# YPares/gaast

Hardware: AMD Instinct MI355X
Metric: full-MV geometric products/sec (dim n); achieved HBM GB/s vs roofline (higher is better)
Workload: dtype f32; 1 GPU; R^12 full MV x MV geometric product, f32 (BASELINE configs[2]); dim=12, batch_per_gpu=65536, global_batch=65536

## Files before the change

gaast_amd/csrc/device/kernels_dense.hip.hpp:

```cpp
#pragma once
#include "kernels_common.hip.hpp"


namespace gaast {

template <typename T>
struct DenseArgs {
    const T* left;
    const T* right;
    T* out;
    int64_t left_stride, right_stride, out_stride;
    const uint32_t* left_map;
    const uint32_t* right_map;
    int left_count, right_count;
    int left_full, right_full;
    int left_contig, right_contig;
    const int32_t* out_map;
    int canon_left, canon_right;
    int n;
    uint32_t neg_hi, zero_hi;
    uint32_t neg_lo;
    int beta;
    const T* left_scale;
    const T* right_scale;
// ... 275 lines not shown
        asm("v_pk_fma_f32 %0, %1, %2, %0 op_sel:[1,1,0] op_sel_hi:[1,0,1]" : "+v"(c) : "v"(a), "v"(b));
    else if constexpr (X == 1 && NL == 1 && NH == 0)
        asm("v_pk_fma_f32 %0, %1, %2, %0 op_sel:[1,1,0] op_sel_hi:[1,0,1] neg_lo:[1,0,0]" : "+v"(c) : "v"(a), "v"(b));
    else if constexpr (X == 1 && NL == 0 && NH == 1)
        asm("v_pk_fma_f32 %0, %1, %2, %0 op_sel:[1,1,0] op_sel_hi:[1,0,1] neg_hi:[1,0,0]" : "+v"(c) : "v"(a), "v"(b));
    else
        asm("v_pk_fma_f32 %0, %1, %2, %0 op_sel:[1,1,0] op_sel_hi:[1,0,1] neg_lo:[1,0,0] neg_hi:[1,0,0]" : "+v"(c) : "v"(a), "v"(b));
}

template <bool ODD, bool NEGLO, int IDX>
__device__ __forceinline__ void gp_block16_pk(const float2v (&A2)[8], const float2v (&B2)[8], float2v (&C2)[8]) {
    if constexpr (IDX < 128) {
        constexpr int a = IDX >> 3, j = IDX & 7, c0 = 2 * j;
        constexpr int b_lo = a ^ c0, b_hi = a ^ c0 ^ 1;
        constexpr int nl = lo_reorder_parity(a, b_lo) ^ (ODD ? (__builtin_popcount(b_lo) & 1) : 0) ^
                           (NEGLO ? (__builtin_popcount(a & b_lo) & 1) : 0);
        constexpr int nh = lo_reorder_parity(a, b_hi) ^ (ODD ? (__builtin_popcount(b_hi) & 1) : 0) ^
                           (NEGLO ? (__builtin_popcount(a & b_hi) & 1) : 0);
        pk_fma_sel<(a & 1), nl, nh>(C2[j], A2[a >> 1], B2[b_lo >> 1]);
        gp_block16_pk<ODD, NEGLO, IDX + 1>(A2, B2, C2);
    }
}

template <typename T>
struct BlockStep;

template <>
struct BlockStep<float> {
    float2v C2[8];
    __device__ __forceinline__ void init() {
#pragma unroll
        for (int i = 0; i < 8; ++i) C2[i] = float2v{0.f, 0.f};
    }
    template <bool ODD, bool NEGLO>
    __device__ __forceinline__ void step(const float* As, const float* Bs, int a_hi, int b_hi, float sgn) {
        const int sa = (a_hi >> 2) & 3, sb = (b_hi >> 2) & 3;
        const float4v* ap = reinterpret_cast<const float4v*>(As + (a_hi << 4));
        const float4v* bp = reinterpret_cast<const float4v*>(Bs + (b_hi << 4));
        float2v A2[8], B2[8];
        const float2v s2 = float2v{sgn, sgn};
#pragma unroll
        for (int q = 0; q < 4; ++q) {
            const float4v va = ap[q ^ sa];
            const float4v vb = bp[q ^ sb];
            A2[2 * q] = float2v{va.x, va.y};
            A2[2 * q + 1] = float2v{va.z, va.w};
            B2[2 * q] = float2v{vb.x, vb.y} * s2;
            B2[2 * q + 1] = float2v{vb.z, vb.w} * s2;
        }
        gp_block16_pk<ODD, NEGLO, 0>(A2, B2, C2);
    }
    __device__ __forceinline__ float get(int i) const { return (i & 1) ? C2[i >> 1].y : C2[i >> 1].x; }
};

template <>
struct BlockStep<double> {
    double C[16];
    __device__ __forceinline__ void init() {
#pragma unroll
        for (int i = 0; i < 16; ++i) C[i] = 0.0;
    }
    template <bool ODD, bool NEGLO>
    __device__ __forceinline__ void step(const double* As, const double* Bs, int a_hi, int b_hi, double sgn) {
        const int sa = (a_hi >> 2) & 3, sb = (b_hi >> 2) & 3;
        const double2v* ap = reinterpret_cast<const double2v*>(As + (a_hi << 4));
        const double2v* bp = reinterpret_cast<const double2v*>(Bs + (b_hi << 4));
        double A[16], B[16];
#pragma unroll
        for (int q = 0; q < 4; ++q) {
            const double2v a0 = ap[2 * (q ^ sa)], a1 = ap[2 * (q ^ sa) + 1];
            const double2v b0 = bp[2 * (q ^ sb)], b1 = bp[2 * (q ^ sb) + 1];
            A[4 * q + 0] = a0.x; A[4 * q + 1] = a0.y; A[4 * q + 2] = a1.x; A[4 * q + 3] = a1.y;
            B[4 * q + 0] = b0.x * sgn; B[4 * q + 1] = b0.y * sgn; B[4 * q + 2] = b1.x * sgn; B[4 * q + 3] = b1.y * sgn;
        }
        gp_block16<double, ODD, NEGLO>(A, B, C);
    }
    __device__ __forceinline__ double get(int i) const { return C[i]; }
};

template <typename T, bool DEGENERATE, int THREADS, bool NEGLO, bool SCALED = false, bool CHAINED = false>
__global__ __launch_bounds__(THREADS) void k_gp_dense(DenseArgs<T> p) {
    const T* const left_scale = SCALED ? p.left_scale : nullptr;
    const T* const right_scale = SCALED ? p.right_scale : nullptr;
    const T* const out_scale = SCALED ? p.out_scale : nullptr;
    extern __shared__ __attribute__((aligned(16))) unsigned char smem_raw[];
    T* smem = reinterpret_cast<T*>(smem_raw);
    const int n = p.n;
    const int N = 1 << n;
    const int hbits = n - 4;
    const int LPI = 1 << hbits;
    const int IPB = THREADS >> hbits;
    const int item_stride = 2 * N + (IPB > 1 ? 4 : 0);
    const int tid = threadIdx.x;
    const T zero = T(0);
    const int64_t num_groups = (p.batch + IPB - 1) / IPB;

    const int it = tid >> hbits;
    const int c_hi = tid & (LPI - 1);
    int32_t om[16];
#pragma unroll
    for (int i = 0; i < 16; ++i) om[i] = p.out_map[(c_hi << 4) + i];

    for (int64_t grp = blockIdx.x; grp < num_groups; grp += gridDim.x) {
        const int64_t item0 = grp * IPB;
        const int nitems = int(p.batch - item0 < IPB ? p.batch - item0 : IPB);
        {
            if (!p.left_full || !p.right_full) {
                for (int i = tid; i < nitems * item_stride; i += THREADS) smem[i] = zero;
                __syncthreads();
            }
            if constexpr (CHAINED)
                stage_from_list<T, THREADS>(p, item0, nitems, smem, item_stride, smem + p.pre_scratch, tid);
            else
                stage_operands<T, THREADS>(p.left + item0 * p.left_stride, p.left_stride, p.left_map, p.left_count, p.left_contig,
                                           p.canon_left, smem, item_stride, nitems, tid, left_scale);
            stage_operands<T, THREADS>(p.right + item0 * p.right_stride, p.right_stride, p.right_map, p.right_count,
                                       p.right_contig, p.canon_right, smem + N, item_stride, nitems, tid, right_scale);
        }
        __syncthreads();

        if (it < nitems) {
            const T* As = smem + it * item_stride;
            const T* Bs = As + N;
            BlockStep<T> acc;
            acc.init();

            auto one_step = [&](auto odd_tag, int a_hi) {
                constexpr bool ODD = decltype(odd_tag)::value;
                uint32_t sp = uint32_t(a_hi) >> 1;
                sp ^= sp >> 1;
                sp ^= sp >> 2;
                sp ^= sp >> 4;
                sp ^= sp >> 8;
                const uint32_t M = sp ^ (uint32_t(a_hi) & p.neg_hi);
                const uint32_t u = (__builtin_popcount(uint32_t(a_hi) & sp) ^
                                    __builtin_popcount(uint32_t(a_hi) & p.neg_hi)) & 1u;
                const uint32_t sbit = (u ^ uint32_t(__builtin_popcount(uint32_t(c_hi) & M))) & 1u;
                T sgn = sbit ? T(-1) : T(1);
                if (DEGENERATE) {
                    if (uint32_t(a_hi) & ~uint32_t(c_hi) & p.zero_hi) sgn = zero;
                }
                acc.template step<ODD, NEGLO>(As, Bs, a_hi, a_hi ^ c_hi, sgn);
            };
            const int half = LPI >> 1;
            for (int i = 0; i < half; ++i) one_step(std::false_type{}, (i << 1) | (__builtin_popcount(uint32_t(i)) & 1));
            for (int i = 0; i < half; ++i) one_step(std::true_type{}, (i << 1) | ((__builtin_popcount(uint32_t(i)) & 1) ^ 1));

            T* orow = p.out + (item0 + it) * p.out_stride;
#pragma unroll
            for (int i = 0; i < 16; ++i) store_result<T>(orow, om[i], acc.get(i), p.beta, out_scale, (c_hi << 4) + i);
        }
        __syncthreads();
    }
}


__device__ __forceinline__ constexpr int lo5_reorder_parity(int a, int b) {
    int par = 0;
    for (int p = 1; p < 5; ++p)
        if ((a >> p) & 1)
            for (int q = 0; q < p; ++q) par ^= (b >> q) & 1;
    return par;
}

__device__ __forceinline__ int mfma_b_pos(int m) {
    const int x = m >> 5, k = m & 31;
    const int lq = ((k & 1) << 2) | (k >> 3);
    return (x << 5) | (((lq ^ (x >> 1)) & 7) << 2) | ((k >> 1) & 3);
}

template <bool DEGENERATE, int THREADS, bool SCALED = false, bool CHAINED = false>
__global__ __launch_bounds__(THREADS) void k_gp_mfma32(DenseArgs<float> p) {
    const float* const left_scale = SCALED ? p.left_scale : nullptr;
    const float* const right_scale = SCALED ? p.right_scale : nullptr;
    const float* const out_scale = SCALED ? p.out_scale : nullptr;
    extern __shared__ __attribute__((aligned(16))) unsigned char smem_raw[];
    float* smem = reinterpret_cast<float*>(smem_raw);
    const int n = p.n;
    const int N = 1 << n;
    const int hbits = n - 5;
    const int H = 1 << hbits;
    const int WPI = H >> 5;
    const int IPB = (THREADS >> 6) / WPI;
    const int item_stride = 2 * N;
    const int tid = threadIdx.x;
    const int64_t item0 = int64_t(blockIdx.x) * IPB;
    const int nitems = int(p.batch - item0 < IPB ? p.batch - item0 : IPB);

    if (!p.left_full || !p.right_full) {
        for (int i = tid; i < nitems * item_stride; i += THREADS) smem[i] = 0.f;
        __syncthreads();
    }
    {
        if constexpr (CHAINED)
            stage_from_list<float, THREADS>(p, item0, nitems, smem, item_stride, smem + p.pre_scratch, tid);
        else
            stage_operands<float, THREADS>(p.left + item0 * p.left_stride, p.left_stride, p.left_map, p.left_count, p.left_contig,
                                       p.canon_left, smem, item_stride, nitems, tid, left_scale);
        stage_operands<float, THREADS>(p.right + item0 * p.right_stride, p.right_stride, p.right_map, p.right_count,
                                       p.right_contig, p.canon_right, smem + N, item_stride, nitems, tid, right_scale);
    }
    __syncthreads();

    const int wave = tid >> 6, lane = tid & 63;
    const int it = wave / WPI, tile = wave - it * WPI;
    if (it < nitems) {
        const float* As = smem + it * item_stride;
        const float* Bs = As + N;
        const int i = lane & 31, h = lane >> 5;
        const int c_hi = (tile << 5) | i;

        uint32_t amask[16];
        uint32_t aoff[16];
#pragma unroll
        for (int s2 = 0; s2 < 16; ++s2) {
            const int k = 2 * s2 + h;
            const int a_lo = i ^ k;
            int par = __builtin_popcount(uint32_t(a_lo & k) & p.neg_lo) & 1;
            for (int pp = 1; pp < 5; ++pp)
                if ((a_lo >> pp) & 1) par ^= __builtin_popcount(k & ((1 << pp) - 1)) & 1;
            amask[s2] = uint32_t(par) << 31;
            aoff[s2] = uint32_t(a_lo) << 2;
        }

        float16v acc;
#pragma unroll
        for (int r = 0; r < 16; ++r) acc[r] = 0.f;

        const unsigned char* As_b = reinterpret_cast<const unsigned char*>(As);
        const unsigned char* Bs_b = reinterpret_cast<const unsigned char*>(Bs);
        uint32_t bq[4];
#pragma unroll
        for (int q = 0; q < 4; ++q) bq[q] = (uint32_t(c_hi) << 7) | (uint32_t((((h << 2) | q) ^ (c_hi >> 1)) & 7) << 4);
        const uint32_t c_hi_u = uint32_t(c_hi) | 0x8000u;
        auto one_step = [&](int a_hi) {
            uint32_t sp = uint32_t(a_hi) >> 1;
            sp ^= sp >> 1;
            sp ^= sp >> 2;
            sp ^= sp >> 4;
            sp ^= sp >> 8;
            const uint32_t M = sp ^ (uint32_t(a_hi) & p.neg_hi);
            const uint32_t u = (__builtin_popcount(uint32_t(a_hi) & sp) ^
                                __builtin_popcount(uint32_t(a_hi) & p.neg_hi)) & 1u;
            const uint32_t bmask = uint32_t(__builtin_popcount(c_hi_u & (M | (u << 15)))) << 31;
            float bscale = 1.f;
            if (DEGENERATE) {
                if (uint32_t(a_hi) & ~uint32_t(c_hi) & p.zero_hi) bscale = 0.f;
            }
            float bv[16];
            const uint32_t sx = (uint32_t(a_hi) << 7) | (uint32_t((a_hi >> 1) & 7) << 4);
#pragma unroll
            for (int q = 0; q < 4; ++q) {
                const float4v v = *reinterpret_cast<const float4v*>(Bs_b + (bq[q] ^ sx));
                bv[4 * q + 0] = v.x; bv[4 * q + 1] = v.y; bv[4 * q + 2] = v.z; bv[4 * q + 3] = v.w;
            }
            const uint32_t abase = uint32_t(a_hi) << 7;
#pragma unroll
            for (int s2 = 0; s2 < 16; ++s2) {
                float a = *reinterpret_cast<const float*>(As_b + abase + aoff[s2]);
                a = __uint_as_float(__float_as_uint(a) ^ amask[s2]);
                float b = __uint_as_float(__float_as_uint(bv[s2]) ^ bmask);
                if (DEGENERATE) b *= bscale;
                acc = __builtin_amdgcn_mfma_f32_32x32x2f32(a, b, acc, 0, 0, 0);
            }
        };
        const int half = H >> 1;
        for (int t2 = 0; t2 < half; ++t2) one_step((t2 << 1) | (__builtin_popcount(uint32_t(t2)) & 1));
#pragma unroll
        for (int s2 = 0; s2 < 16; ++s2)
            amask[s2] ^= uint32_t((__builtin_popcount(uint32_t(s2)) + h) & 1) << 31;
        for (int t2 = 0; t2 < half; ++t2) one_step((t2 << 1) | ((__builtin_popcount(uint32_t(t2)) & 1) ^ 1));

        float* orow = p.out + (item0 + it) * p.out_stride;
        const int32_t* om = p.out_map + (c_hi << 5);
#pragma unroll
        for (int r = 0; r < 16; ++r) {
            const int c_lo = (r & 3) + 8 * (r >> 2) + 4 * h;
            store_result<float>(orow, om[c_lo], acc[r], p.beta, out_scale, (c_hi << 5) + c_lo);
        }
    }
}

template <int THREADS>
__device__ __forceinline__ void lds_barrier() {
    if (THREADS <= 64) {
        __builtin_amdgcn_wave_barrier();
        asm volatile("" ::: "memory");
    } else {
        asm volatile("s_waitcnt lgkmcnt(0)\n\ts_barrier" ::: "memory");
    }
}

typedef __attribute__((address_space(3))) unsigned char lds_u8;
typedef uint32_t uint4v __attribute__((ext_vector_type(4)));

__device__ __forceinline__ uint32_t xor3(uint32_t a, uint32_t b, uint32_t c) {
#if __has_builtin(__builtin_amdgcn_bitop3_b32)
    return __builtin_amdgcn_bitop3_b32(a, b, c, 0x96);
#else
    return a ^ b ^ c;
#endif
}

__device__ __forceinline__ constexpr int mfma16_k(int t) {
    constexpr int order[16] = {0, 3, 5, 6, 9, 10, 12, 15, 1, 2, 4, 7, 8, 11, 13, 14};
    return order[t];
}

template <bool DEGENERATE, int NDIM, bool SCALED = false, bool CHAINED = false>
__global__ __launch_bounds__(NDIM == 13 ? 512 : 256, NDIM <= 11 ? 2 : 1) void k_gp_mfma32p(DenseArgs<float> p) {
    const float* const left_scale = SCALED ? p.left_scale : nullptr;
    const float* const right_scale = SCALED ? p.right_scale : nullptr;
    const float* const out_scale = SCALED ? p.out_scale : nullptr;
    extern __shared__ __attribute__((aligned(16))) unsigned char smem_raw[];
    float* smem = reinterpret_cast<float*>(smem_raw);
    lds_u8* lds = (lds_u8*)smem_raw;
    constexpr int n = NDIM;
    constexpr int THREADS = NDIM == 13 ? 512 : 256;
    constexpr int N = 1 << n;
    constexpr int H = 1 << (n - 5);
    constexpr int WPI = H >> 5;
    constexpr int IPB = (THREADS >> 6) / WPI;
    constexpr int item_stride = 4 * N;
    constexpr uint32_t NEG = uint32_t(N) << 2;
    constexpr int PR = N / 4;
    constexpr int MPR = PR / THREADS;
    constexpr int ROWS = 2 * IPB;
    static_assert(MPR * ROWS == 8, "eight 16-byte pieces per thread and group");
    const int tid = threadIdx.x;
    const int64_t num_groups = (p.batch + IPB - 1) / IPB;
    const bool fast = !SCALED && !CHAINED && p.left_contig && p.right_contig && p.left_full && p.right_full;

    if (tid < 16) smem[IPB * item_stride + tid] = 0.f;

    uint32_t mw[2][MPR * 4];
    float4 pf[8];
    auto fetch = [&](int64_t g) {
        const int64_t it0 = g * IPB;
        const int cnt = int(p.batch - it0 < IPB ? p.batch - it0 : IPB);
#pragma unroll
        for (int r = 0; r < ROWS; ++r) {
            const int k = r % IPB;
            if (k < cnt) {
                const float* row = r < IPB ? p.left + (it0 + k) * p.left_stride : p.right + (it0 + k) * p.right_stride;
#pragma unroll
                for (int m = 0; m < MPR; ++m) pf[r * MPR + m] = reinterpret_cast<const float4*>(row)[tid + m * THREADS];
            }
        }
    };
    if (fast) {
#pragma unroll
        for (int m = 0; m < MPR; ++m) {
            const uint4 ml = reinterpret_cast<const uint4*>(p.left_map)[tid + m * THREADS];
            const uint4 mr = reinterpret_cast<const uint4*>(p.right_map)[tid + m * THREADS];
            mw[0][4 * m + 0] = ml.x; mw[0][4 * m + 1] = ml.y; mw[0][4 * m + 2] = ml.z; mw[0][4 * m + 3] = ml.w;
            mw[1][4 * m + 0] = mr.x; mw[1][4 * m + 1] = mr.y; mw[1][4 * m + 2] = mr.z; mw[1][4 * m + 3] = mr.w;
        }
        if (int64_t(blockIdx.x) < num_groups) fetch(blockIdx.x);
    }

    const int wave = tid >> 6, lane = tid & 63;
    const int it = wave / WPI, tile = wave - it * WPI;
    const int i = lane & 31, h = lane >> 5;
    const int c_hi = (tile << 5) | i;
    const uint32_t item_base = uint32_t(it) * uint32_t(item_stride) * 4u;

    constexpr bool ABS_A = NDIM <= 11 || (NDIM == 12 && !DEGENERATE);
    const uint32_t lds0 = ABS_A ? uint32_t(size_t(lds)) : 0u;
    uint32_t ak0[16];
#pragma unroll
    for (int t = 0; t < 16; ++t) {
        const int k = 2 * mfma16_k(t) + h;
        const int a_lo = i ^ k;
        int par = __builtin_popcount(uint32_t(a_lo & k) & p.neg_lo) & 1;
        for (int pp = 1; pp < 5; ++pp)
            if ((a_lo >> pp) & 1) par ^= __builtin_popcount(k & ((1 << pp) - 1)) & 1;
        ak0[t] = lds0 + item_base + (uint32_t(a_lo) << 2) + (par ? NEG : 0u);
    }
    const uint32_t b_base = item_base + 2u * NEG;
    constexpr uint32_t zero_block = uint32_t(IPB) * uint32_t(item_stride) * 4u;
    uint32_t bq[4];
#pragma unroll
    for (int q = 0; q < 4; ++q) {
        bq[q] = (uint32_t(c_hi) << 7) | (uint32_t((((h << 2) | q) ^ (c_hi >> 1)) & 7) << 4);
        if ((__builtin_popcount(uint32_t(c_hi)) & 1) && (((q >> 1) ^ h) & 1)) bq[q] ^= NEG;
    }
    const uint32_t c_hi_u = uint32_t(c_hi) | 0x8000u;
    auto sign_terms = [&](int a_hi, uint32_t& M, uint32_t& u) {
        uint32_t sp = uint32_t(a_hi) >> 1;
        sp ^= sp >> 1;
        sp ^= sp >> 2;
        sp ^= sp >> 4;
        sp ^= sp >> 8;
        M = sp ^ (uint32_t(a_hi) & p.neg_hi);
        u = (__builtin_popcount(uint32_t(a_hi) & sp) ^ __builtin_popcount(uint32_t(a_hi) & p.neg_hi)) & 1u;
    };
    auto block_sign = [&](int a_hi) -> uint32_t {
        uint32_t M, u;
        sign_terms(a_hi, M, u);
        return uint32_t(__builtin_popcount(c_hi_u & (M | (u << 15)))) & 1u;
    };
    constexpr int SIGN_WORDS = H <= 64 ? H / 32 : 0;
    constexpr bool XOR_STEP = NDIM == 12 && !DEGENERATE;
    if (XOR_STEP && (lds0 & ((16u << n) - 1u))) __builtin_trap();
    uint32_t dlt[XOR_STEP ? 7 : 1] = {0};
    uint32_t ud[XOR_STEP ? H / 32 : 1] = {0};
    if constexpr (XOR_STEP) {
#pragma unroll
        for (int t = 0; t < 7; ++t) {
            const uint32_t P = (2u << t) - 1u;
            uint32_t M, u;
            sign_terms(int(P), M, u);
            dlt[t] = (P << 7) ^ (((P >> 1) & 7u) << 4) ^ ((uint32_t(__builtin_popcount(uint32_t(c_hi) & M)) & 1u) << (n + 2));
        }
#pragma unroll
        for (int w = 0; w < H / 32; ++w) {
            uint32_t bits = 0;
#pragma unroll 1
            for (int b = 0; b < 32; ++b) {
                uint32_t M, u0, u1;
                sign_terms(32 * w + b, M, u0);
                sign_terms(32 * w + b + 1, M, u1);
                bits |= (u0 ^ u1) << b;
            }
            ud[w] = __builtin_amdgcn_readfirstlane(bits);
        }
    }
    uint32_t sgn[SIGN_WORDS > 0 ? SIGN_WORDS : 1] = {0};
#pragma unroll
    for (int w = 0; w < SIGN_WORDS; ++w) {
        uint32_t bits = 0;
#pragma unroll 1
        for (int b = 0; b < 32; ++b) bits |= block_sign(32 * w + b) << b;
        sgn[w] = bits;
    }

    for (int64_t g = blockIdx.x; g < num_groups; g += gridDim.x) {
        const int64_t item0 = g * IPB;
        const int nitems = int(p.batch - item0 < IPB ? p.batch - item0 : IPB);
        if (fast) {
            auto stage_row = [&](int r, bool canon) {
                const int k = r % IPB, side = r / IPB;
                if (k < nitems) {
#pragma unroll
                    for (int m = 0; m < MPR; ++m) {
                        const float4 v = pf[r * MPR + m];
                        const float x[4] = {v.x, v.y, v.z, v.w};
#pragma unroll
                        for (int c = 0; c < 4; ++c) {
                            const uint32_t w = mw[side][4 * m + c];
                            float y = x[c];
                            if (canon) y = 0.f + y;
                            const uint32_t yb = __float_as_uint(y) ^ (w & 0x80000000u);
                            const uint32_t at = uint32_t(k) * uint32_t(item_stride * 4) + (side ? 2u * NEG : 0u) + (((w >> 16) & 0x7fffu) << 2);
                            *(__attribute__((address_space(3))) uint32_t*)(lds + at) = yb;
                            *(__attribute__((address_space(3))) uint32_t*)(lds + at + NEG) = yb ^ 0x80000000u;
                        }
                    }
                }
            };
#pragma unroll
            for (int r = 0; r < ROWS; ++r) {
                if constexpr (XOR_STEP) {
                    if (r / IPB ? p.canon_right : p.canon_left) stage_row(r, true);
                    else stage_row(r, false);
                } else {
                    stage_row(r, r / IPB ? p.canon_right : p.canon_left);
                }
            }
        } else {
            if (!p.left_full || !p.right_full) {
                for (int e = tid; e < nitems * item_stride; e += THREADS) smem[e] = 0.f;
                lds_barrier<THREADS>();
            }
            if constexpr (CHAINED)
                stage_from_list<float, THREADS>(p, item0, nitems, smem, item_stride, smem + p.pre_scratch, tid);
            else
                stage_operands<float, THREADS>(p.left + item0 * p.left_stride, p.left_stride, p.left_map, p.left_count, p.left_contig,
                                           p.canon_left, smem, item_stride, nitems, tid, left_scale);
            stage_operands<float, THREADS>(p.right + item0 * p.right_stride, p.right_stride, p.right_map, p.right_count,
                                           p.right_contig, p.canon_right, smem + 2 * N, item_stride, nitems, tid, right_scale);
            lds_barrier<THREADS>();
            constexpr int quads_per_item = N >> 1;
            for (int e = tid; e < nitems * quads_per_item; e += THREADS) {
                const int sit = e / quads_per_item, j = e - sit * quads_per_item;
                const int src = sit * item_stride + (j << 2) + ((j << 2) < N ? 0 : N);
                const float4v v = *reinterpret_cast<const float4v*>(smem + src);
                *reinterpret_cast<float4v*>(smem + src + N) = -v;
            }
        }
        lds_barrier<THREADS>();
        if (fast && g + gridDim.x < num_groups) fetch(g + gridDim.x);

        if (it < nitems) {
            float16v acc;
#pragma unroll
            for (int r = 0; r < 16; ++r) acc[r] = 0.f;
            uint32_t akc[XOR_STEP ? 1 : 16];
            uint32_t (&ak)[16] = *reinterpret_cast<uint32_t (*)[16]>(XOR_STEP ? ak0 : akc);
            if constexpr (!XOR_STEP) {
#pragma unroll
                for (int t = 0; t < 16; ++t) ak[t] = ak0[t];
            }

            auto step = [&](int a_hi, int j, uint32_t sxs) {
                uint32_t bw[16], aw[16];
#pragma unroll
                for (int q = 0; q < 4; ++q) {
                    uint32_t addr = b_base + (bq[q] ^ sxs);
                    if (DEGENERATE) addr = (uint32_t(a_hi) & ~uint32_t(c_hi) & p.zero_hi) ? zero_block : addr;
                    const uint4v v = *(__attribute__((address_space(3))) const uint4v*)(lds + addr);
                    bw[4 * q + 0] = v.x; bw[4 * q + 1] = v.y; bw[4 * q + 2] = v.z; bw[4 * q + 3] = v.w;
                }
#pragma unroll
                for (int t = 0; t < 16; ++t)
                    aw[t] = ABS_A ? *(__attribute__((address_space(3))) const uint32_t*)size_t(ak[t] + uint32_t(j << 7))
                                  : *(__attribute__((address_space(3))) const uint32_t*)(lds + ak[t] + uint32_t(j << 7));
#pragma unroll
                for (int t = 0; t < 16; ++t)
                    acc = __builtin_amdgcn_mfma_f32_32x32x2f32(__uint_as_float(aw[t]), __uint_as_float(bw[t]), acc, 0, 0, 0);
                asm volatile("" ::: "memory");
            };
            if constexpr (SIGN_WORDS > 0 && NDIM <= 11) {
                uint32_t awin[4];
                uint4v qb[2];
                auto b_quad = [&](int a_hi, int q, uint32_t sxs) -> uint4v {
                    uint32_t addr = b_base + (bq[q] ^ sxs);
                    if (DEGENERATE) addr = (uint32_t(a_hi) & ~uint32_t(c_hi) & p.zero_hi) ? zero_block : addr;
                    return *(__attribute__((address_space(3))) const uint4v*)(lds + addr);
                };
                auto a_word = [&](int t, int j) -> uint32_t {
                    return ABS_A ? *(__attribute__((address_space(3))) const uint32_t*)size_t(ak[t] + uint32_t(j << 7))
                                 : *(__attribute__((address_space(3))) const uint32_t*)(lds + ak[t] + uint32_t(j << 7));
                };
                auto sx_of = [&](int a_hi) -> uint32_t {
                    uint32_t sx = __builtin_amdgcn_readfirstlane((uint32_t(a_hi) << 7) | (uint32_t((a_hi >> 1) & 7) << 4));
                    asm("" : "+s"(sx));
                    return sx;
                };
                uint32_t sxs = ((sgn[0] & 1u) << (n + 2)) | sx_of(0);
                qb[0] = b_quad(0, 0, sxs);
#pragma unroll
                for (int t = 0; t < 3; ++t) awin[t] = a_word(t, 0);
#pragma unroll
                for (int w = 0; w < SIGN_WORDS; ++w) {
                    uint32_t sw = sgn[w];
                    const uint32_t next_word_bit0 = w + 1 < SIGN_WORDS ? (sgn[w + 1 < SIGN_WORDS ? w + 1 : w] & 1u) : 0u;
#pragma unroll 1
                    for (int c = 0; c < 2; ++c) {
                        const int a0 = 32 * w + 16 * c;
#pragma unroll
                        for (int j = 0; j < 16; ++j) {
                            const int a_hi = a0 + j;
                            const uint32_t nbit = j < 15 ? (sw >> (j + 1)) & 1u : (c == 0 ? (sw >> 16) & 1u : next_word_bit0);
                            const uint32_t nsxs = (nbit << (n + 2)) | sx_of(a_hi + 1);
#pragma unroll
                            for (int t = 0; t < 16; ++t) {
                                const int m = 16 * j + t;
                                const int t3 = (t + 3) & 15, j3 = j + ((t + 3) >> 4);
                                awin[(m + 3) & 3] = a_word(t3, j3);
                                if ((t & 3) == 0) {
                                    const int q = t >> 2;
                                    qb[(q + 1) & 1] = q < 3 ? b_quad(a_hi, q + 1, sxs) : b_quad(a_hi + 1, 0, nsxs);
                                }
                                __builtin_amdgcn_sched_barrier(0);
                                const uint4v bqv = qb[(t >> 2) & 1];
                                const uint32_t bwv = (t & 3) == 0 ? bqv.x : (t & 3) == 1 ? bqv.y : (t & 3) == 2 ? bqv.z : bqv.w;
                                acc = __builtin_amdgcn_mfma_f32_32x32x2f32(__uint_as_float(awin[m & 3]), __uint_as_float(bwv), acc, 0, 0, 0);
                                __builtin_amdgcn_sched_barrier(0);
                            }
                            sxs = nsxs;
                        }
                        sw >>= 16;
#pragma unroll
                        for (int t = 0; t < 16; ++t) ak[t] += 16u << 7;
                    }
                }
            } else if constexpr (XOR_STEP) {
                uint32_t xb[4];
#pragma unroll
                for (int q = 0; q < 4; ++q) xb[q] = lds0 + (b_base | bq[q]);
#pragma unroll 1
                for (int c = 0; c < H / 64; ++c) {
                    const uint32_t udw[2] = {c == 0 ? ud[0] : ud[2], c == 0 ? ud[1] : ud[3]};
#pragma unroll
                    for (int j = 0; j < 64; ++j) {
                        uint32_t bw[16], aw[16];
#pragma unroll
                        for (int q = 0; q < 4; ++q) {
                            const uint4v v = *(__attribute__((address_space(3))) const uint4v*)size_t(xb[q]);
                            bw[4 * q + 0] = v.x; bw[4 * q + 1] = v.y; bw[4 * q + 2] = v.z; bw[4 * q + 3] = v.w;
                        }
#pragma unroll
                        for (int t = 0; t < 16; ++t)
                            aw[t] = *(__attribute__((address_space(3))) const uint32_t*)size_t(ak[t] + uint32_t(j << 7));
#pragma unroll
                        for (int t = 0; t < 16; ++t)
                            acc = __builtin_amdgcn_mfma_f32_32x32x2f32(__uint_as_float(aw[t]), __uint_as_float(bw[t]), acc, 0, 0, 0);
                        asm volatile("" ::: "memory");
                        uint32_t su = __builtin_amdgcn_readfirstlane(((udw[j >> 5] >> (j & 31)) & 1u) << (n + 2));
                        asm("" : "+s"(su));
                        const uint32_t d = dlt[j < 63 ? __builtin_ctz(~uint32_t(j)) : 6];
#pragma unroll
                        for (int q = 0; q < 4; ++q) xb[q] = xor3(xb[q], d, su);
                    }
#pragma unroll
                    for (int t = 0; t < 16; ++t) ak[t] ^= 64u << 7;
                }
            } else {
                for (int a0 = 0; a0 < H; a0 += 8) {
#pragma unroll
                    for (int j = 0; j < 8; ++j) {
                        const int a_hi = a0 + j;
                        const uint32_t sx = (uint32_t(a_hi) << 7) | (uint32_t((a_hi >> 1) & 7) << 4);
                        step(a_hi, j, (block_sign(a_hi) << (n + 2)) | sx);
                    }
#pragma unroll
                    for (int t = 0; t < 16; ++t) ak[t] += 8u << 7;
                }
            }

            float* orow = p.out + (item0 + it) * p.out_stride;
            if constexpr (XOR_STEP) {
                const int32_t* om = p.out_map + (c_hi << 5);
                int32_t ow[16];
#pragma unroll
                for (int r = 0; r < 16; ++r) ow[r] = om[(r & 3) + 8 * (r >> 2) + 4 * h];
                asm volatile("" ::: "memory");
                auto put = [&](bool signs, bool beta) {
#pragma unroll
                    for (int r = 0; r < 16; ++r) {
                        const int32_t w = ow[r];
                        if (w < 0) continue;
                        float v = acc[r];
                        if (out_scale) v = v * out_scale[(c_hi << 5) + (r & 3) + 8 * (r >> 2) + 4 * h];
                        if (signs && (w & 0x40000000)) v = beta ? -v : 0.f + (-v);
                        float* dst = orow + (signs ? w & 0x3fffffff : w);
                        *dst = beta ? *dst + v : v;
                    }
                };
                if (p.out_signs) put(true, p.beta != 0);
                else put(false, p.beta != 0);
            } else {
                const int32_t* om = p.out_map + (c_hi << 5);
#pragma unroll
                for (int r = 0; r < 16; ++r) {
                    const int c_lo = (r & 3) + 8 * (r >> 2) + 4 * h;
                    store_result<float>(orow, om[c_lo], acc[r], p.beta, out_scale, (c_hi << 5) + c_lo);
                }
            }
        }
        lds_barrier<THREADS>();
    }
}

typedef double double4m __attribute__((ext_vector_type(4)));

template <typename T>
struct Mfma16x4;
template <>
struct Mfma16x4<double> {
    typedef double4m acc_t;
    static constexpr int SHIFT = 3;
    static __device__ __forceinline__ acc_t mma(double a, double b, acc_t c) { return __builtin_amdgcn_mfma_f64_16x16x4f64(a, b, c, 0, 0, 0); }
    static __device__ __forceinline__ int row(int kq, int r) { return 4 * r + kq; }
    static constexpr bool QUAD = false;
    static __device__ __forceinline__ constexpr int k_of(int kq, int s) { return 4 * s + kq; }
    static __device__ __forceinline__ double flip(double v, uint32_t bit31) { return __hiloint2double(__double2hiint(v) ^ int(bit31), __double2loint(v)); }
};
template <>
struct Mfma16x4<float> {
    typedef float4v acc_t;
    static constexpr int SHIFT = 2;
    static __device__ __forceinline__ acc_t mma(float a, float b, acc_t c) { return __builtin_amdgcn_mfma_f32_16x16x4f32(a, b, c, 0, 0, 0); }
    static __device__ __forceinline__ int row(int kq, int r) { return 4 * kq + r; }
    static constexpr bool QUAD = true;
    static __device__ __forceinline__ constexpr int k_of(int kq, int s) {
        constexpr int tab[4][4] = {{0, 3, 5, 6}, {9, 10, 12, 15}, {1, 2, 4, 7}, {8, 11, 13, 14}};
        return tab[kq][s];
    }
    static __device__ __forceinline__ float flip(float v, uint32_t bit31) { return __uint_as_float(__float_as_uint(v) ^ bit31); }
};

template <typename T, bool DEGENERATE, int NDIM, int MODE, bool SCALED = false, bool CHAINED = false>
__global__ __launch_bounds__(64 << (NDIM - 8)) __attribute__((amdgpu_waves_per_eu(2))) void k_gp_mfma16x4(DenseArgs<T> p) {
    constexpr bool FAST = MODE >= 1;
    static_assert(!(SCALED && MODE != 0), "a rescaled basis runs on the general staging and stores");
    const T* const left_scale = SCALED ? p.left_scale : nullptr;
    const T* const right_scale = SCALED ? p.right_scale : nullptr;
    const T* const out_scale = SCALED ? p.out_scale : nullptr;
    extern __shared__ __attribute__((aligned(16))) unsigned char smem_raw[];
    T* smem = reinterpret_cast<T*>(smem_raw);
    lds_u8* lds = (lds_u8*)smem_raw;
    typedef __attribute__((address_space(3))) T lds_t;
    typedef Mfma16x4<T> MM;
    constexpr int ES = MM::SHIFT;
    constexpr int n = NDIM;
    constexpr int N = 1 << n;
    constexpr int H = 1 << (n - 4);
    constexpr int THREADS = 64 << (n - 8);
#ifndef GAAST_MFMA16X4_PAD_MAXN
#define GAAST_MFMA16X4_PAD_MAXN 9
#endif
    constexpr int PAD_A = NDIM <= GAAST_MFMA16X4_PAD_MAXN ? 16 : 0;
    constexpr int A_EL = PAD_A ? 2 * N : 0, B_EL = PAD_A ? 0 : 2 * N;
    constexpr int item_stride = 4 * N + 32;
    constexpr uint32_t NEG = uint32_t(N) << ES;
    constexpr uint32_t A_BASE = uint32_t(A_EL) << ES, NEG_A = uint32_t(N + PAD_A) << ES;
    constexpr uint32_t B_BASE = uint32_t(B_EL) << ES;
    constexpr int BS = 4 + ES;
    const int tid = threadIdx.x;
    if (tid < 16) smem[4 * N + PAD_A + tid] = T(0);

    const int tile = tid >> 6, lane = tid & 63;
    const int i = lane & 15, kq = lane >> 4;
    const int c_hi = (tile << 4) | i;

    uint32_t ak[4], bk[4];
#pragma unroll
    for (int s = 0; s < 4; ++s) {
        const int k = MM::k_of(kq, s);
        const int a_lo = i ^ k;
        int par = __builtin_popcount(uint32_t(a_lo & k) & p.neg_lo) & 1;
        for (int pp = 1; pp < 4; ++pp)
            if ((a_lo >> pp) & 1) par ^= __builtin_popcount(k & ((1 << pp) - 1)) & 1;
        ak[s] = A_BASE + (uint32_t(a_lo) << ES) + (par ? NEG_A : 0u);
        if (MM::QUAD) {
            bk[s] = (uint32_t(c_hi) << BS) | (uint32_t(kq ^ (((c_hi >> 2) & 1) << 1)) << 4);
            if ((__builtin_popcount(uint32_t(c_hi)) & 1) && kq >= 2) bk[s] ^= NEG;
        } else {
            bk[s] = (uint32_t(c_hi) << BS) | ((uint32_t((c_hi >> 1) & 7) << (1 + ES)) ^ (uint32_t(k) << ES));
            if ((__builtin_popcount(uint32_t(c_hi)) & __builtin_popcount(uint32_t(k))) & 1) bk[s] ^= NEG;
        }
    }
    constexpr int SW = (H + 31) / 32, SB = H < 32 ? H : 32;
    uint32_t sign_bits[SW], zero_bits[SW];
#pragma unroll
    for (int w = 0; w < SW; ++w) {
        uint32_t sb = 0, zb = 0;
#pragma unroll 1
        for (int b = 0; b < SB; ++b) {
            const int a_hi = 32 * w + b;
            uint32_t sp = uint32_t(a_hi) >> 1;
            sp ^= sp >> 1;
            sp ^= sp >> 2;
            sp ^= sp >> 4;
            const uint32_t M = sp ^ (uint32_t(a_hi) & p.neg_hi);
            const uint32_t u = (__builtin_popcount(uint32_t(a_hi) & sp) ^ __builtin_popcount(uint32_t(a_hi) & p.neg_hi)) & 1u;
            sb |= ((u ^ uint32_t(__builtin_popcount(uint32_t(c_hi) & M))) & 1u) << b;
            if (DEGENERATE) zb |= ((uint32_t(a_hi) & ~uint32_t(c_hi) & p.zero_hi) ? 1u : 0u) << b;
        }
        sign_bits[w] = sb;
        zero_bits[w] = zb;
    }
    constexpr uint32_t zero_block = uint32_t(4 * N + PAD_A) << ES;
#pragma unroll
    for (int s = 0; s < 4; ++s) bk[s] |= B_BASE;
    uint32_t ooff[4], osg[4];
    bool ook[4];
    T osc[4];
#pragma unroll
    for (int r = 0; r < 4; ++r) {
        const int32_t w = p.out_map[(c_hi << 4) + MM::row(kq, r)];
        ook[r] = w >= 0;
        ooff[r] = uint32_t(w & 0x3fffffff) << ES;
        osg[r] = (uint32_t(w) & 0x40000000u) << 1;
        osc[r] = (SCALED && out_scale) ? out_scale[(c_hi << 4) + MM::row(kq, r)] : T(1);
    }

    constexpr int CPP = 16 >> ES;
    constexpr int PPT = 4 / CPP;
    static_assert((N / CPP) == PPT * THREADS, "four components of each row per thread");
    uint32_t wa[4] = {0, 0, 0, 0}, wb[4] = {0, 0, 0, 0}, sa[4] = {0, 0, 0, 0}, sb[4] = {0, 0, 0, 0};
    T pf_l[4], pf_r[4];
    const bool same_src = CHAINED && p.pre_left == p.right && p.pre_left_stride == p.right_stride && p.pre_left_len == N &&
                          p.pre_right_len <= THREADS;
    T pf_x = T(0);
    auto fetch = [&](int64_t item) {
#pragma unroll
        for (int m = 0; m < PPT; ++m) {
            uint32_t o = uint32_t(tid + m * THREADS) * 16u;
            asm volatile("" : "+v"(o));
            if constexpr (!CHAINED) {
                const uint4 xl = *reinterpret_cast<const uint4*>(reinterpret_cast<const unsigned char*>(p.left + item * p.left_stride) + o);
                __builtin_memcpy(&pf_l[m * CPP], &xl, 16);
            }
            const uint4 xr = *reinterpret_cast<const uint4*>(reinterpret_cast<const unsigned char*>(p.right + item * p.right_stride) + o);
            __builtin_memcpy(&pf_r[m * CPP], &xr, 16);
        }
        if constexpr (CHAINED) {
            if (same_src && tid < p.pre_right_len) pf_x = p.pre_right[item * p.pre_right_stride + tid];
        }
    };
    if (FAST) {
#pragma unroll
        for (int e = 0; e < 4; ++e) {
            const int idx = ((e / CPP) * THREADS + tid) * CPP + (e % CPP);
            const uint32_t mr = p.right_map[idx];
            if constexpr (!CHAINED) {
                const uint32_t ml = p.left_map[idx];
                wa[e] = A_BASE + (((ml >> 16) & 0x7fffu) << ES);
                sa[e] = ml & 0x80000000u;
            }
            wb[e] = B_BASE + (((mr >> 16) & 0x7fffu) << ES);
            sb[e] = mr & 0x80000000u;
        }
        if (int64_t(blockIdx.x) < p.batch) fetch(blockIdx.x);
    }

    constexpr bool LIST_CACHE = CHAINED && FAST && (NDIM == 8 || NDIM == 9);
    constexpr bool LC_PACKED = NDIM != 8;
    constexpr int LW = NDIM + 1;
    bool list_cached = LIST_CACHE && same_src && p.pre_width == 12 && p.pre_rows == 4 * THREADS && p.pre_row_scale == nullptr;
    uint32_t ce[(LIST_CACHE && LC_PACKED) ? 4 : 1][(LIST_CACHE && LC_PACKED) ? LW : 1];
    const lds_t *cl[(LIST_CACHE && !LC_PACKED) ? 4 : 1][(LIST_CACHE && !LC_PACKED) ? LW : 1], *cr[(LIST_CACHE && !LC_PACKED) ? 4 : 1][(LIST_CACHE && !LC_PACKED) ? LW : 1];
    uint32_t crow[4] = {0, 0, 0, 0};
    if constexpr (LIST_CACHE) {
        if (list_cached) {
            const uint32_t ll = uint32_t(p.pre_left_len), rl = uint32_t(p.pre_right_len);
            bool pads_only = true;
#pragma unroll
            for (int rr = 0; rr < 4; ++rr) {
                crow[rr] = p.pre_row_map[tid + rr * THREADS];
#pragma unroll
                for (int t = 0; t < 12; ++t) {
                    const uint32_t e = p.pre_entries[t * (4 * THREADS) + tid + rr * THREADS];
                    if (t < LW) {
                        const uint32_t la = (uint32_t(p.pre_scratch) + (e & 0x7fffu)) << ES;
                        const uint32_t ra = (uint32_t(p.pre_scratch) + ll + ((e >> 16) & 0x7fffu) + ((e >> 31) ? rl + 1u : 0u)) << ES;
                        if constexpr (LC_PACKED) {
                            ce[rr][t < LW ? t : 0] = la | (ra << 16);
                        } else {
                            cl[rr][t < LW ? t : 0] = (const lds_t*)(lds + la);
                            cr[rr][t < LW ? t : 0] = (const lds_t*)(lds + ra);
                        }
                    } else {
                        pads_only = pads_only && (e & 0x7fffu) == ll + rl;
                    }
                }
            }
            list_cached = __all(pads_only) != 0;
        }
    }
    auto cached_list = [&]() {
        if constexpr (LIST_CACHE) {
#pragma unroll
            for (int rr = 0; rr < 4; ++rr) {
                T lv[LW], rv[LW];
#pragma unroll
                for (int t = 0; t < LW; ++t) {
                    if constexpr (LC_PACKED) {
                        uint32_t e = ce[rr][t];
                        asm volatile("" : "+v"(e));
                        lv[t] = *(const lds_t*)(lds + (e & 0xffffu));
                        rv[t] = *(const lds_t*)(lds + (e >> 16));
                    } else {
                        lv[t] = *cl[rr][t];
                        rv[t] = *cr[rr][t];
                    }
                }
                T acc = T(0);
#pragma unroll
                for (int t = 0; t < LW; ++t) acc = acc + lv[t] * rv[t];
                uint32_t w = crow[rr];
                asm volatile("" : "+v"(w));
                const uint32_t pos = (w >> 16) & 0x7fffu;
                const T val = list_flip<T>(acc, w & 0x80000000u);
                smem[A_EL + pos] = val;
                smem[A_EL + pos + N + PAD_A] = -val;
            }
        }
    };
    for (int64_t item = blockIdx.x; item < p.batch; item += gridDim.x) {
        if (FAST) {
#pragma unroll
            for (int e = 0; e < 4; ++e) {
                T yr = pf_r[e];
                if constexpr (CHAINED) {
                    if (same_src) {
                        const int idx = ((e / CPP) * THREADS + tid) * CPP + (e % CPP);
                        smem[p.pre_scratch + idx] = p.pre_canon_left ? T(0) + yr : yr;
                    }
                } else {
                    T yl = pf_l[e];
                    if (p.left_signs) yl = MM::flip(yl, sa[e]);
                    *(lds_t*)(lds + wa[e]) = yl;
                    *(lds_t*)(lds + wa[e] + NEG_A) = -yl;
                }
                yr = MM::flip(yr, sb[e]);
                *(lds_t*)(lds + wb[e]) = yr;
                *(lds_t*)(lds + wb[e] + NEG) = -yr;
            }
            if constexpr (CHAINED) {
                if (same_src) {
                    if (tid < p.pre_right_len) {
                        const T x = p.pre_canon_right ? T(0) + pf_x : pf_x;
                        smem[p.pre_scratch + N + tid] = x;
                        smem[p.pre_scratch + N + p.pre_right_len + 1 + tid] = -x;
                    }
                    if (tid == 0) smem[p.pre_scratch + N + p.pre_right_len] = T(0);
                } else {
                    list_fill_scratch<T, THREADS>(p, item, 1, smem + p.pre_scratch, tid);
                }
                if (!p.left_full) {
                    for (int e = tid; e < N; e += THREADS) {
                        smem[A_EL + e] = T(0);
                        smem[A_EL + N + PAD_A + e] = T(0);
// ... 447 lines not shown
```

Baseline: 4.307 million products/s.

## Software-pipeline LDS loads with MFMA and compile-time sign masks in R12 XOR path

Reworks the n=12 XOR-step inner loop so A words and B quads are prefetched a few MFMAs ahead in a rotating window, interleaved with each MFMA behind sched_barriers. Before, all 20 LDS loads of a step were issued and then 16 MFMAs ran. The per-step sign-flip bits, which used to be computed at runtime into readfirstlane'd words, now come from a constexpr parity function of j, with runtime selection only when the two chunks differ. The neg_hi contribution is folded into the dlt deltas. This hides LDS latency behind matrix work and removes scalar setup, at the cost of rigid scheduling and more register pressure.

```diff
diff --git a/gaast_amd/csrc/device/kernels_dense.hip.hpp b/gaast_amd/csrc/device/kernels_dense.hip.hpp
--- a/gaast_amd/csrc/device/kernels_dense.hip.hpp
+++ b/gaast_amd/csrc/device/kernels_dense.hip.hpp
@@ -601,6 +601,12 @@
 #endif
 }
 
+__device__ __forceinline__ constexpr bool r12_u0(int a) {
+    int w = 0;
+    for (int b = 0; b < 8; ++b) w += (a >> b) & 1;
+    return (w >> 1) & 1;
+}
+
 __device__ __forceinline__ constexpr int mfma16_k(int t) {
     constexpr int order[16] = {0, 3, 5, 6, 9, 10, 12, 15, 1, 2, 4, 7, 8, 11, 13, 14};
     return order[t];
@@ -703,26 +709,14 @@
     constexpr bool XOR_STEP = NDIM == 12 && !DEGENERATE;
     if (XOR_STEP && (lds0 & ((16u << n) - 1u))) __builtin_trap();
     uint32_t dlt[XOR_STEP ? 7 : 1] = {0};
-    uint32_t ud[XOR_STEP ? H / 32 : 1] = {0};
     if constexpr (XOR_STEP) {
 #pragma unroll
         for (int t = 0; t < 7; ++t) {
             const uint32_t P = (2u << t) - 1u;
             uint32_t M, u;
             sign_terms(int(P), M, u);
-            dlt[t] = (P << 7) ^ (((P >> 1) & 7u) << 4) ^ ((uint32_t(__builtin_popcount(uint32_t(c_hi) & M)) & 1u) << (n + 2));
-        }
-#pragma unroll
-        for (int w = 0; w < H / 32; ++w) {
-            uint32_t bits = 0;
-#pragma unroll 1
-            for (int b = 0; b < 32; ++b) {
-                uint32_t M, u0, u1;
-                sign_terms(32 * w + b, M, u0);
-                sign_terms(32 * w + b + 1, M, u1);
-                bits |= (u0 ^ u1) << b;
-            }
-            ud[w] = __builtin_amdgcn_readfirstlane(bits);
+            const uint32_t par = uint32_t(__builtin_popcount(uint32_t(c_hi) & M) ^ __builtin_popcount(P & p.neg_hi)) & 1u;
+            dlt[t] = (P << 7) ^ (((P >> 1) & 7u) << 4) ^ (par << (n + 2));
         }
     }
     uint32_t sgn[SIGN_WORDS > 0 ? SIGN_WORDS : 1] = {0};
@@ -879,29 +873,41 @@
                 uint32_t xb[4];
 #pragma unroll
                 for (int q = 0; q < 4; ++q) xb[q] = lds0 + (b_base | bq[q]);
+                uint32_t awin[4];
+                uint4v qb[2];
+                auto a_word = [&](int t, int j) -> uint32_t {
+                    return *(__attribute__((address_space(3))) const uint32_t*)size_t(ak[t] + uint32_t(j << 7));
+                };
+                auto b_quad = [&](uint32_t addr) -> uint4v { return *(__attribute__((address_space(3))) const uint4v*)size_t(addr); };
+                qb[0] = b_quad(xb[0]);
+#pragma unroll
+                for (int t = 0; t < 3; ++t) awin[t] = a_word(t, 0);
 #pragma unroll 1
                 for (int c = 0; c < H / 64; ++c) {
-                    const uint32_t udw[2] = {c == 0 ? ud[0] : ud[2], c == 0 ? ud[1] : ud[3]};
+                    uint32_t su_c1 = c ? NEG : 0u, su_c0 = c ? 0u : NEG;
+                    asm("" : "+s"(su_c1), "+s"(su_c0));
 #pragma unroll
                     for (int j = 0; j < 64; ++j) {
-                        uint32_t bw[16], aw[16];
-#pragma unroll
-                        for (int q = 0; q < 4; ++q) {
-                            const uint4v v = *(__attribute__((address_space(3))) const uint4v*)size_t(xb[q]);
-                            bw[4 * q + 0] = v.x; bw[4 * q + 1] = v.y; bw[4 * q + 2] = v.z; bw[4 * q + 3] = v.w;
+                        const uint32_t d = dlt[j < 63 ? __builtin_ctz(~uint32_t(j)) : 6];
+                        const bool m0 = r12_u0(j) != r12_u0(j + 1), m1 = j < 63 ? r12_u0(64 + j) != r12_u0(65 + j) : m0;
+                        const uint32_t su = m0 == m1 ? (m0 ? NEG : 0u) : m1 ? su_c1 : su_c0;
+#pragma unroll
+                        for (int t = 0; t < 16; ++t) {
+                            const int m = 16 * j + t;
+                            const int t3 = (t + 3) & 15, j3 = j + ((t + 3) >> 4);
+                            awin[(m + 3) & 3] = a_word(t3, j3);
+                            if (t == 2) xb[0] = xor3(xb[0], d, su);
+                            if ((t & 3) == 0) {
+                                const int q = ((t >> 2) + 1) & 3;
+                                qb[q & 1] = b_quad(xb[q]);
+                                if (q) xb[q] = xor3(xb[q], d, su);
+                            }
+                            __builtin_amdgcn_sched_barrier(0);
+                            const uint4v bqv = qb[(t >> 2) & 1];
+                            const uint32_t bwv = (t & 3) == 0 ? bqv.x : (t & 3) == 1 ? bqv.y : (t & 3) == 2 ? bqv.z : bqv.w;
+                            acc = __builtin_amdgcn_mfma_f32_32x32x2f32(__uint_as_float(awin[m & 3]), __uint_as_float(bwv), acc, 0, 0, 0);
+                            __builtin_amdgcn_sched_barrier(0);
                         }
-#pragma unroll
-                        for (int t = 0; t < 16; ++t)
-                            aw[t] = *(__attribute__((address_space(3))) const uint32_t*)size_t(ak[t] + uint32_t(j << 7));
-#pragma unroll
-                        for (int t = 0; t < 16; ++t)
-                            acc = __builtin_amdgcn_mfma_f32_32x32x2f32(__uint_as_float(aw[t]), __uint_as_float(bw[t]), acc, 0, 0, 0);
-                        asm volatile("" ::: "memory");
-                        uint32_t su = __builtin_amdgcn_readfirstlane(((udw[j >> 5] >> (j & 31)) & 1u) << (n + 2));
-                        asm("" : "+s"(su));
-                        const uint32_t d = dlt[j < 63 ? __builtin_ctz(~uint32_t(j)) : 6];
-#pragma unroll
-                        for (int q = 0; q < 4; ++q) xb[q] = xor3(xb[q], d, su);
                     }
 #pragma unroll
                     for (int t = 0; t < 16; ++t) ak[t] ^= 64u << 7;
```

Result: no change. 4.346 million products/s (median of 6 runs) (+0.9%).
